# ARPA-SIMC/CRITERIA3D

Measured on AMD Instinct MI355X. Metric: simulated-hours/sec on 512x512x20 grid, higher is better.
Workload: dtype f64

## Files before the change

### criteria3d_amd/csrc/sf3d_control.inc

```

#define SYS_STORE(p, x) __hip_atomic_store((p), (x), __ATOMIC_RELAXED, __HIP_MEMORY_SCOPE_SYSTEM)
#define SYS_LOAD(p) __hip_atomic_load((p), __ATOMIC_RELAXED, __HIP_MEMORY_SCOPE_SYSTEM)

__device__ __forceinline__ unsigned long long rec_lo(double x, uint32_t tag) { return ((unsigned long long)__double_as_longlong(x) & 0xFFFFFFFFull) | ((unsigned long long)tag << 32); }
__device__ __forceinline__ unsigned long long rec_hi(double x, uint32_t tag) { return ((unsigned long long)__double_as_longlong(x) >> 32) | ((unsigned long long)tag << 32); }
__device__ __forceinline__ bool rec_ok(unsigned long long a, unsigned long long b, uint32_t tag) { return (uint32_t)(a >> 32) == tag && (uint32_t)(b >> 32) == tag; }
__device__ __forceinline__ double rec_value(unsigned long long a, unsigned long long b) { return __longlong_as_double((long long)((a & 0xFFFFFFFFull) | (b << 32))); }

__device__ __forceinline__ void dist_combine(double (&acc)[4], const double (&x)[4], int K, int op, bool first)
{
    if (first) { for (int k = 0; k < K; ++k) acc[k] = x[k]; return; }
    if (op == 1) { for (int k = 0; k < K; ++k) acc[k] = dmax(acc[k], x[k]); return; }
    if (op >= 2) {
        dd_merge(acc[0], acc[1], x[0], x[1]);
        if (op == 3) dd_merge(acc[2], acc[3], x[2], x[3]); else for (int k = 2; k < K; ++k) acc[k] += x[k];
        return;
    }
    for (int k = 0; k < K; ++k) acc[k] += x[k];
}
template <int K>
__device__ __forceinline__ bool dist_allgather(const DevView& v, Ctrl* c, double (&vals)[K], int op)
{
    static_assert(K >= 1 && K <= 4, "a mailbox holds four values");
    if (v.world <= 1) return true;
// ... 245 lines not shown
__device__ __forceinline__ void begin_attempt(Ctrl* c)
{
    c->dt = dmin(c->dtCurr, c->maxTimeStep);
    c->hold = c->cur;
    c->best = -1;
    c->bestMBR = NODATA_D;
    c->approx = 0;
    c->counters[0]++;
    c->stage = ST_APPROX;
}

__global__ void k_step_begin(Ctrl* c, double maxTimeStep)
{
    c->maxTimeStep = maxTimeStep;
    c->seqCount = 0;
    c->aBuf ^= 1u;
    begin_attempt(c);
}

__device__ __forceinline__ void reject_attempt(Ctrl* c)
{
    c->seSource = 2;
    c->cur = c->hold;
    begin_attempt(c);
}

#ifndef SF3D_PROBE_BUDGET
#define SF3D_PROBE_BUDGET 8u
#endif
__device__ __forceinline__ void courant_decision(Ctrl* c, double cmax)
{
// ... 172 lines not shown
```

### criteria3d_amd/csrc/sf3d_device.h

```cpp
#ifndef SF3D_DEVICE_H
#define SF3D_DEVICE_H

#include <stdint.h>

#define SF3D_SLOTS 10
#define SF3D_POOL 5
#define SF3D_BLOCK 256
#define SF3D_CHUNK 64
#define SF3D_MAX_BLOCKS 2048
#define CK_NONE 0
#define CK_MIXED 255

enum : uint8_t { LK_NONE = 0, LK_SOIL_VERT = 1, LK_SOIL_LAT = 2, LK_RUNOFF = 3, LK_INFILTRATION = 4 };

enum : uint32_t {
    ST_IDLE = 0,
    ST_ATTEMPT = 1,
    ST_APPROX = 2,
    ST_SWEEP = 3,
    ST_POST = 4,
    ST_RESTORE = 5,
    ST_ACCEPT = 6,
    ST_DONE = 7,
    ST_FAIL = 8
// ... 48 lines not shown
    double courant;
    double bestMBR;
    double bestNorm;
    double lastNorm;
    uint32_t stage, approx, iter, iterBudget;
    int32_t cur, hold, best;
    uint32_t linearValid;
    uint32_t seSource;
    uint32_t epoch;
    uint32_t distError;
    uint32_t distSilent;
    uint32_t pairRecTimeout;
    uint32_t kfEpoch, haloEpoch, haloPar; int32_t haloBuf;
    int32_t acceptBuf;
    uint32_t aBuf, acceptABuf;
    double acceptDt;
    BalanceDev curStep, prevStep, curPeriod, wholePeriod;
    uint32_t hStage, hIter, hIterBudget, hRows;
    int32_t tCur, tOld;
    uint32_t hSweepsLast, hPad;
    double dtWater;
    double hOuterDt, hOuterSum;
    double hMaxStep, hDt, hDone;
    double hCourant, hNorm;
    double hCacheDt;
    unsigned long long hNormBits;
    HeatBalanceDev heatCur, heatPrev;
    double heatPeriodSink;
    double query[2];
    uint32_t lineal;
// ... 109 lines not shown
    const uint32_t* nodeLat;
    const uint64_t* chunkCode;
    unsigned int* bar;
    unsigned long long* rec;
    unsigned long long* prec;
    unsigned long long* gpub;
    unsigned long long* prec2;
    uint32_t fusedPost;
    double* pub;
    const uint32_t* haloSrc;
    uint32_t forceTimeout;
    int32_t sidePeer[2];
    uint32_t recFast, putBase[2];
};

struct DevView {
    uint32_t N, ns, nb;
    uint32_t Nnorm;
    uint32_t nChunks;
    uint32_t qSplit;
    uint32_t nbSurf, nbSoil;
    double probeMin;
    const uint32_t* chunkList; uint32_t nList, nListSurf;
    const uint32_t* asmList;
    uint32_t pLo, pHi;
    uint32_t aLo, aHi;
    const uint32_t* bndList; uint32_t nBnd;
    const uint16_t* lmask;
    uint32_t haloDirect;
    uint32_t ntStream;
    const DistView* dist;
    int32_t world, rank;
    const uint8_t* owner;
    const ChunkDesc* cdesc;
    const double *z, *size, *pond, *sink;
    const uint16_t* cls;
    const uint8_t* btype;
    const double *bslope, *bsize, *prescribed;
    const uint32_t* lto;
    const uint8_t* lkind;
    const uint8_t* probeMask;
    const double *larea, *ldist;
    double* lflowSum;
    sf3d_d2* A2x[2];
    double *b, *C;
    double* X[SF3D_POOL];
    double *Se, *SeHold, *K, *flow, *bflowRate, *bflowSum;
    double* compatCv; uint8_t* compatCn; double* compatDiag;
    double *cgDiag, *cgR, *cgP, *cgQ;
    double *part0, *part1;
    double *part2, *part3;
    unsigned int* arrive;
    unsigned int* gridBar;
    const SoilDev* soils;
    const double* roughness;
    PairGrid pair;
    ResGrid res;
    Ctrl* ctrl;
    HeatDev heat;
// ... 262 lines not shown
```

### criteria3d_amd/csrc/sf3d_host_build.inc

```

namespace {

template <class F> void parallel_for(uint32_t n, F f)
{
    unsigned nt = std::thread::hardware_concurrency();
    if (nt == 0) nt = 1;
    if (nt > 16) nt = 16;
    if (n < 65536 || nt == 1) { f(0u, n); return; }
    std::vector<std::thread> th;
    const uint32_t chunk = (n + nt - 1) / nt;
    for (unsigned t = 0; t < nt; ++t) {
        const uint32_t a = t * chunk, b = (a + chunk < n) ? a + chunk : n;
        if (a >= b) break;
        th.emplace_back([=] { f(a, b); });
    }
    for (auto& t : th) t.join();
}

const char* kKernelNames[KID_COUNT] = {"k_props", "k_assemble", "k_sweep", "k_post", "k_restore", "k_accept", "k_sweep_pair", "k_sweep_resident", "k_output_map"};

}

sf3d_error_t sf3d_partition_bounds(uint32_t ns, int world, uint32_t* bounds)
{
// ... 130 lines not shown
    char* tables = nullptr;
    double* nodes = nullptr;
    size_t off[8] = {0};
    uint32_t nCells = 0, nrLayers = 0, nUnits = 0, nSoils = 0, nodesN = 0;
    uint64_t nodesColVer = 0;
    int32_t lastEvapLayer = 0;
    double area = 0.;
    float flag = -9999.f;
    bool computed = false;
    double lastMs = 0.;
};

struct DeviceSolver::Impl {
    int device = -1;
    hipStream_t stream = nullptr;
    hipStream_t stream2 = nullptr;
    hipEvent_t evLinks[2] = {nullptr, nullptr};
    bool linksPending[2] = {false, false};
    int overlapAccept = -1;
    DevView v{};
    Ctrl* hostCtrl = nullptr;
    std::vector<void*> allocs;
    uint32_t N = 0, ns = 0;
    uint32_t ownedNodes = 0;
    uint32_t lastSweeps = 8;
    uint32_t lastBatches = 1;
    uint32_t predCount = 0, pred[16] = {0};
    uint32_t lastHeatSweeps = 8;
    std::vector<uint32_t> gsLevelStart;
    uint32_t lastHeatSteps = 1;
    double* heatOut[6] = {nullptr};
    double* heatAirP = nullptr;
    std::vector<std::pair<uint32_t, hipGraphExec_t>> graphs;
    int useFused = -1;
// ... 45 lines not shown
        SF3D_SYM(pGroupStart, "ncclGroupStart"); SF3D_SYM(pGroupEnd, "ncclGroupEnd"); SF3D_SYM(pAllGather, "ncclAllGather");
        #undef SF3D_SYM
        return true;
    }
    void rccl_halo(hipStream_t st, int fields)
    {
        pGroupStart();
        for (int p = 0; p < hostDist.world; ++p) {
            if (p == hostDist.rank) continue;
            if (hostDist.sendCount[p]) pSend(hostDist.sendBuf[p], (size_t)hostDist.sendCount[p] * fields, ncclDouble, p, comm, st);
            if (hostDist.recvCount[p]) pRecv(const_cast<double*>(hostDist.recvBuf[p]), (size_t)hostDist.recvCount[p] * fields, ncclDouble, p, comm, st);
        }
        pGroupEnd();
    }
    void rccl_gather(hipStream_t st) { pAllGather(rcclMine, rcclGathered, 4, ncclDouble, comm, st); }
    std::vector<uint8_t> dslot;
    std::vector<double> stage;
    uint32_t connectGen = 0;
    bool warnedShared = false;
    int timing = 0;
    std::vector<std::pair<const void*, uint32_t>> residentBlocks;
    std::vector<uint32_t> propsNeed;
    hipStream_t stream3 = nullptr;
    hipEvent_t evSlab[8] = {};
    int slabs = -1; uint32_t slabPropsBlocks = 0, slabAsmBlocks = 0; double slabFirst = 0.;
    int residentGrids = -1;
    uint32_t pairBlocks = 0;
    bool pairMasked = false;
    uint32_t resBlocks = 0, resLds = 0;
    uint32_t resCapacity = 0;
// ... 37 lines not shown
    if (!impl_) impl_ = new Impl();
    int count = 0;
    HIP_TRY(hipGetDeviceCount(&count));
    if (dev < 0 || dev >= count) { snprintf(err_, sizeof(err_), "device %d out of range (%d visible)", dev, count); return SF3D_SOLVER_ERROR; }
    impl_->device = dev;
    HIP_TRY(hipSetDevice(dev));
    return SF3D_OK;
}

static uint64_t g_deviceBytes = 0;
sf3d_error_t DeviceSolver::release()
{
    if (!impl_) return SF3D_OK;
    Impl& I = *impl_;
    if (I.stream) hipStreamSynchronize(I.stream);
    if (I.stream2) hipStreamSynchronize(I.stream2);
    if (I.stream3) hipStreamSynchronize(I.stream3);
#if SF3D_RES_PROFILE
    if (built_ && I.v.res.on && I.v.res.pub) {
        double pr[32];
        if (hipMemcpy(pr, I.v.res.pub, sizeof(pr), hipMemcpyDeviceToHost) == hipSuccess && pr[16] > 0.) {
            const char* names[7] = {"compute + record stores issued", "wave sum + block partial", "halo records", "partial records of all blocks", "barrier B", "norm + decision", "(prologue: per launch, not per iteration)"};
            fprintf(stderr, "[sf3d] resident sweep loop, block 0: %.0f launches, %.2f iterations per launch, %.2f us per launch\n", pr[16], pr[15] / pr[16], pr[17] / pr[16] / 100.);
            for (int p = 0; p < 7; ++p) fprintf(stderr, "[sf3d]   %-40s %7.2f us per iteration\n", names[p], pr[8 + p] / pr[15] / 100.);
        }
    }
#endif
    I.linksPending[0] = I.linksPending[1] = false;
    if (I.stream3) {
        (void)hipStreamDestroy(I.stream3); I.stream3 = nullptr;
        for (auto& ev : I.evSlab) if (ev) { (void)hipEventDestroy(ev); ev = nullptr; }
    }
    I.slabs = -1;
    for (auto& p : I.pending) { I.freeEvents.push_back(p.a); I.freeEvents.push_back(p.b); }
    I.pending.clear();
    for (auto& g : I.graphs) hipGraphExecDestroy(g.second);
    I.graphs.clear();
    for (void* p : I.allocs) hipFree(p);
    I.allocs.clear();
    g_deviceBytes = 0;
    I.maps.free_all();
    if (I.sink.nodes) { (void)hipFree(I.sink.nodes); I.sink.nodes = nullptr; I.sink.nodesN = 0; I.sink.computed = false; }
    if (I.comm && I.pCommDestroy) { I.pCommDestroy(I.comm); I.comm = nullptr; }
// ... 1 lines not shown
    for (void* p : I.peerMaps) hipIpcCloseMemHandle(p);
    I.peerMaps.clear();
    I.drop_shm();
    if (I.window) { hipFree(I.window); I.window = nullptr; }
    I.devDist = nullptr; I.distStats = nullptr;
    connected_ = false;
    built_ = false;
    fatal_ = false;
    I.overlapAccept = I.useFused = I.useGraphs = I.residentGrids = -1;
    return SF3D_OK;
}

sf3d_error_t DeviceSolver::synchronize()
{
    if (!impl_ || !impl_->stream) return SF3D_OK;
    HIP_TRY(hipStreamSynchronize(impl_->stream));
    if (impl_->stream2) { HIP_TRY(hipStreamSynchronize(impl_->stream2)); impl_->linksPending[0] = impl_->linksPending[1] = false; }
    return SF3D_OK;
}

template <class T> static hipError_t dev_alloc(std::vector<void*>& allocs, T*& p, size_t count)
{
    void* q = nullptr;
    hipError_t e = hipMalloc(&q, (count ? count : 1) * sizeof(T));
    if (e == hipSuccess) { allocs.push_back(q); p = static_cast<T*>(q); g_deviceBytes += (uint64_t)(count ? count : 1) * sizeof(T); }
    return e;
}
uint64_t DeviceSolver::device_bytes() const { return g_deviceBytes; }

static void fill_params(Ctrl& c, const ParamsHost& p)
{
    c.MBRThreshold = p.MBRThreshold; c.residualTolerance = p.residualTolerance;
// ... 22 lines not shown
                if (pick < 0 || pick >= count) { snprintf(err_, sizeof(err_), "SF3D_DEVICES names device %d, %d visible", pick, count); return SF3D_SOLVER_ERROR; }
                dev = pick;
            }
        }
        I.device = dev % count;
    }
    HIP_TRY(hipSetDevice(I.device));
    if (!I.stream) HIP_TRY(hipStreamCreateWithFlags(&I.stream, hipStreamNonBlocking));
    return SF3D_OK;
}

sf3d_error_t DeviceSolver::sync_to_device(HostModel& m, const ParamsHost& p)
{
    { const sf3d_error_t e = ensure_device(); if (e != SF3D_OK) return e; }
    Impl& I = *impl_;
    if ((I.linksPending[0] || I.linksPending[1]) && (m.graphDirty || m.stateDirty || m.flowSumsDirty || !built_)) { HIP_TRY(hipStreamSynchronize(I.stream2)); I.linksPending[0] = I.linksPending[1] = false; }
    if (!I.hostCtrl) HIP_TRY(hipHostMalloc((void**)&I.hostCtrl, sizeof(Ctrl), hipHostMallocDefault));

    const uint32_t N = m.N, ns = m.ns;
    const size_t NS = (size_t)N * SF3D_SLOTS;

    if (m.graphDirty || !built_) {
        if (world_ > 1 && connected_) { snprintf(err_, sizeof(err_), "topology changed after sf3d_dist_connect: call sf3d_dist_prepare / export / connect again"); return SF3D_TOPOGRAPHY_ERROR; }
        if (m.surf.size() < N || m.hasClass.size() < N) { snprintf(err_, sizeof(err_), "the model's build arrays were released (a trimmed strip): re-initialise before changing the topology"); return SF3D_TOPOGRAPHY_ERROR; }
        for (uint32_t i = 0; i < N; ++i) {
            if ((m.surf[i] != 0) != (i < ns)) { snprintf(err_, sizeof(err_), "node %u: surface nodes must be exactly the first nrSurfaceNodes indices", i); return SF3D_TOPOGRAPHY_ERROR; }
            if (!m.hasClass[i]) { snprintf(err_, sizeof(err_), "node %u has no soil/surface class", i); return SF3D_MISSING_DATA_ERROR; }
        }
        if (built_) { if (m.hostStaleState) fetch_state(m); if (m.hostStaleFlows) fetch_flows(m); if (m.heat && m.hostStaleHeat && I.v.heat.on) fetch_heat(m); }
        release();
        I.N = N; I.ns = ns;
// ... 377 lines not shown
            const uint32_t per = SF3D_BLOCK / SF3D_CHUNK;
            auto blocks = [&](uint32_t chunks) { uint32_t b = (chunks + per - 1) / per; if (b > SF3D_MAX_BLOCKS) b = SF3D_MAX_BLOCKS; return b; };
            v.nbSoil = blocks(v.nList - v.nListSurf);
            if (const char* be = getenv("SF3D_ASM_SOIL_BLOCKS")) { const uint32_t nb = (uint32_t)atoi(be); if (nb > 0 && nb < v.nbSoil) v.nbSoil = nb; }
        }
        double *z, *size, *pond, *sink, *bslope, *bsize, *prescribed, *roughness, *larea, *ldist;
        uint16_t* cls; uint8_t *btype, *lkind; uint32_t* lto; SoilDev* soils; ChunkDesc* dcdesc;
        HIP_TRY(dev_alloc(I.allocs, z, N)); HIP_TRY(dev_alloc(I.allocs, size, N));
        HIP_TRY(dev_alloc(I.allocs, pond, N)); HIP_TRY(dev_alloc(I.allocs, sink, N));
        HIP_TRY(dev_alloc(I.allocs, cls, N)); HIP_TRY(dev_alloc(I.allocs, btype, N));
        HIP_TRY(dev_alloc(I.allocs, bslope, N)); HIP_TRY(dev_alloc(I.allocs, bsize, N));
        HIP_TRY(dev_alloc(I.allocs, prescribed, N));
        HIP_TRY(dev_alloc(I.allocs, lto, NS)); HIP_TRY(dev_alloc(I.allocs, lkind, NS));
        HIP_TRY(dev_alloc(I.allocs, larea, NS)); HIP_TRY(dev_alloc(I.allocs, ldist, NS));
        HIP_TRY(dev_alloc(I.allocs, v.lflowSum, NS)); HIP_TRY(dev_alloc(I.allocs, v.A2x[0], NS / 2)); HIP_TRY(dev_alloc(I.allocs, v.A2x[1], NS / 2));
        HIP_TRY(dev_alloc(I.allocs, v.b, N)); HIP_TRY(dev_alloc(I.allocs, v.C, N));
        for (int k = 0; k < SF3D_POOL; ++k) HIP_TRY(dev_alloc(I.allocs, v.X[k], N));
        HIP_TRY(dev_alloc(I.allocs, v.Se, N)); HIP_TRY(dev_alloc(I.allocs, v.K, N)); HIP_TRY(dev_alloc(I.allocs, v.SeHold, N));
        HIP_TRY(dev_alloc(I.allocs, dcdesc, (size_t)nChunks));
        uint32_t* dlist; HIP_TRY(dev_alloc(I.allocs, dlist, listSurf.size()));
        if (!listSurf.empty()) HIP_TRY(hipMemcpy(dlist, listSurf.data(), listSurf.size() * 4, hipMemcpyHostToDevice));
        v.chunkList = dlist;
        v.asmList = dlist;
        v.owner = nullptr; v.dist = nullptr;
        {
            const char* e = getenv("SF3D_NT_STREAM");
            const double sweepBytes = 152.0 * (double)v.nList * SF3D_CHUNK;
            v.ntStream = e ? (e[0] != '0') : (sweepBytes > 256.0 * 1024 * 1024);
        }
        {
// ... 566 lines not shown
                for (uint32_t i = 0; i < ns; ++i) if (kind[(size_t)sl * N + i] == LK_RUNOFF) { v.probeMin = -1.; break; }
            uint8_t* dpm; HIP_TRY(dev_alloc(I.allocs, dpm, (size_t)(ns ? ns : 1)));
            if (ns) HIP_TRY(hipMemcpy(dpm, pm.data(), ns, hipMemcpyHostToDevice));
            v.probeMask = dpm;
        }
        {   std::vector<uint16_t> mask(N, 0);
            for (int sl = 0; sl < SF3D_SLOTS; ++sl) { const uint8_t* kk = kind.data() + (size_t)sl * N; for (uint32_t i = 0; i < N; ++i) if (kk[i] != LK_NONE) mask[i] |= (uint16_t)(1u << sl); }
            uint16_t* dm; HIP_TRY(dev_alloc(I.allocs, dm, N));
            HIP_TRY(hipMemcpy(dm, mask.data(), (size_t)N * 2, hipMemcpyHostToDevice));
            v.lmask = dm; }
        HIP_TRY(hipMemcpy(larea, area.data(), NS * 8, hipMemcpyHostToDevice));
        HIP_TRY(hipMemcpy(ldist, dist.data(), NS * 8, hipMemcpyHostToDevice));
        HIP_TRY(hipMemcpy(dcdesc, cdesc.data(), cdesc.size() * sizeof(ChunkDesc), hipMemcpyHostToDevice));
        if (!sd.empty()) HIP_TRY(hipMemcpy(soils, sd.data(), sd.size() * sizeof(SoilDev), hipMemcpyHostToDevice));
        if (!m.roughness.empty()) HIP_TRY(hipMemcpy(roughness, m.roughness.data(), m.roughness.size() * 8, hipMemcpyHostToDevice));
        HIP_TRY(hipMemset(v.A2x[0], 0, NS * 8)); HIP_TRY(hipMemset(v.A2x[1], 0, NS * 8)); HIP_TRY(hipMemset(v.b, 0, N * 8)); HIP_TRY(hipMemset(v.C, 0, N * 8));
        HIP_TRY(hipMemset(v.flow, 0, N * 8)); HIP_TRY(hipMemset(v.bflowRate, 0, N * 8)); HIP_TRY(hipMemset(v.SeHold, 0, N * 8));
        for (int k = 0; k < SF3D_POOL; ++k) HIP_TRY(hipMemset(v.X[k], 0, N * 8));
        if (m.heat && I.heatAirP) hipLaunchKernelGGL(k_heat_static, dim3(v.nb), dim3(SF3D_BLOCK), 0, 0, v, I.heatAirP);
        HIP_TRY(hipDeviceSynchronize());

        std::memset(&mirror_, 0, sizeof(mirror_));
        mirror_.cur = 0; mirror_.hold = 0; mirror_.best = -1; mirror_.stage = ST_IDLE;
        mirror_.bestMBR = NODATA_D;
        mirror_.tCur = 0; mirror_.tOld = 0; mirror_.hStage = HS_IDLE;
        built_ = true;
        m.graphDirty = false;
        m.stateDirty = m.sinkDirty = m.pondDirty = m.boundaryDirty = m.flowSumsDirty = m.ctrlDirty = true;
        m.sinkLo = 0; m.sinkHi = UINT32_MAX;
        m.hostStaleState = m.hostStaleFlows = false;
    }

    DevView& v = I.v;
    if (m.stateDirty) {
        HIP_TRY(hipMemcpyAsync(v.X[mirror_.cur], m.H.data(), N * 8, hipMemcpyHostToDevice, I.stream));
        HIP_TRY(hipMemcpyAsync(v.Se, m.Se.data(), N * 8, hipMemcpyHostToDevice, I.stream));
        HIP_TRY(hipMemcpyAsync(v.K, m.K.data(), N * 8, hipMemcpyHostToDevice, I.stream));
        mirror_.seSource = 0; m.ctrlDirty = true;
        m.stateDirty = false;
    }
// ... 55 lines not shown
```

### criteria3d_amd/csrc/sf3d_host_step.inc

```
sf3d_error_t DeviceSolver::fetch_state(HostModel& m)
{
    Impl& I = *impl_;
    HIP_TRY(hipMemcpyAsync(m.H.data(), I.v.X[mirror_.cur], (size_t)m.N * 8, hipMemcpyDeviceToHost, I.stream));
    HIP_TRY(hipMemcpyAsync(m.Se.data(), I.v.Se, (size_t)m.N * 8, hipMemcpyDeviceToHost, I.stream));
    HIP_TRY(hipMemcpyAsync(m.K.data(), I.v.K, (size_t)m.N * 8, hipMemcpyDeviceToHost, I.stream));
    HIP_TRY(hipStreamSynchronize(I.stream));
    m.hostStaleState = false;
    return SF3D_OK;
}

sf3d_error_t DeviceSolver::fetch_flows(HostModel& m)
{
    Impl& I = *impl_;
    const size_t N = m.N;
    if (I.stream2) { HIP_TRY(hipStreamSynchronize(I.stream2)); I.linksPending[0] = I.linksPending[1] = false; }
    HIP_TRY(hipMemcpyAsync(m.bflowSum.data(), I.v.bflowSum, N * 8, hipMemcpyDeviceToHost, I.stream));
    HIP_TRY(hipMemcpyAsync(m.bflowRate.data(), I.v.bflowRate, N * 8, hipMemcpyDeviceToHost, I.stream));
    if (I.dslot.empty()) {
        for (int s = 0; s < SF3D_SLOTS; ++s)
            HIP_TRY(hipMemcpyAsync(m.lflowSum[s].data(), I.v.lflowSum + (size_t)s * N, N * 8, hipMemcpyDeviceToHost, I.stream));
        HIP_TRY(hipStreamSynchronize(I.stream));
    } else {
        I.stage.resize(N * SF3D_SLOTS);
        HIP_TRY(hipMemcpyAsync(I.stage.data(), I.v.lflowSum, N * SF3D_SLOTS * 8, hipMemcpyDeviceToHost, I.stream));
        HIP_TRY(hipStreamSynchronize(I.stream));
        for (int s = 0; s < SF3D_SLOTS; ++s) {
            const uint8_t* d = I.dslot.data() + (size_t)s * N; double* dst = m.lflowSum[s].data();
            for (size_t i = 0; i < N; ++i) dst[i] = I.stage[(size_t)d[i] * N + i];
        }
    }
// ... 632 lines not shown
sf3d_error_t DeviceSolver::step(HostModel& m, ParamsHost& p, double maxTimeStep, double* dtOut)
{
    RoctxRange stepRange("sf3d computeStep");
    sf3d_error_t e = sync_to_device(m, p);
    if (e != SF3D_OK) return e;
    if (world_ > 1 && !connected_) { snprintf(err_, sizeof(err_), "multi-GPU model used before sf3d_dist_connect / sf3d_dist_finalize%s%.150s", distWhy_[0] ? ": " : "", distWhy_); return SF3D_SOLVER_ERROR; }
    Impl& I = *impl_;
    const DevView& v = I.v;
    const dim3 grid(v.nb), block(SF3D_BLOCK), one(1);
    const bool multi = world_ > 1;
    const bool heatOn = v.heat.on != 0;
    if (I.useFused < 0) { const char* e = getenv("SF3D_FUSED_DECIDE"); I.useFused = (e && e[0] == '0') ? 0 : 1; }
    if (I.residentGrids < 0) { const char* e = getenv("SF3D_RESIDENT_GRIDS"); I.residentGrids = (e && e[0] == '0') ? 0 : 1; }
    const bool compat = v.compatCv != nullptr;
    auto resident = [&](const void* fn) -> dim3 {
        uint32_t nbk = 0;
        for (auto& r : I.residentBlocks) if (r.first == fn) nbk = r.second;
        if (nbk == 0) {
            int perCu = 0, dev = 0; hipDeviceProp_t prop;
            nbk = SF3D_MAX_BLOCKS;
            if (hipOccupancyMaxActiveBlocksPerMultiprocessor(&perCu, fn, SF3D_BLOCK, 0) == hipSuccess && perCu > 0
                && hipGetDevice(&dev) == hipSuccess && hipGetDeviceProperties(&prop, dev) == hipSuccess && prop.multiProcessorCount > 0)
                nbk = (uint32_t)perCu * (uint32_t)prop.multiProcessorCount;
            if (I.residentGrids == 0) nbk = SF3D_MAX_BLOCKS;
            I.residentBlocks.push_back({fn, nbk});
        }
        return dim3(v.nb < nbk ? v.nb : nbk);
    };
    if (heatOn && multi) I.useFused = 1;
    const bool fused = !multi && I.useFused;
    const bool fusedMulti = multi && I.useFused;
    const bool linealOn = p.lineal && v.cgDiag != nullptr && !multi && I.useFused;
    const bool resOn = v.res.on && I.resBlocks != 0 && (fused || (fusedMulti && v.haloDirect && !I.rcclMode)) && !linealOn;
    if (resOn && !multi) {
        static const long failAt = getenv("SF3D_RESIDENT_FAIL_TEST") ? strtol(getenv("SF3D_RESIDENT_FAIL_TEST"), nullptr, 10) : -1;
        I.v.res.forceTimeout = (failAt >= 0 && (long)I.stepSeqAll == failAt) ? 1u : 0u;
        ++I.stepSeqAll;
    }
    const bool pairOn = !resOn && (fused || (fusedMulti && v.haloDirect && v.nBnd != 0)) && I.pairBlocks != 0 && !linealOn;
    const dim3 pgrid(I.pushBlocks ? I.pushBlocks : 1);
    hipStream_t st = I.stream;

    const bool timedStep = I.timing == 1 || (I.timing == 2 && (I.stepSeq++ % 8 == 0));
    if (I.overlapAccept < 0) { const char* oe = getenv("SF3D_OVERLAP_ACCEPT"); I.overlapAccept = (oe && oe[0] == '0') ? 0 : 1; }
    if (I.overlapAccept && !multi && !I.stream2) { HIP_TRY(hipStreamCreateWithFlags(&I.stream2, hipStreamNonBlocking)); HIP_TRY(hipEventCreateWithFlags(&I.evLinks[0], hipEventDisableTiming)); HIP_TRY(hipEventCreateWithFlags(&I.evLinks[1], hipEventDisableTiming)); }
    const bool overlap = I.overlapAccept && !multi && I.stream2 && !timedStep && I.timing != 1 && v.compatCv == nullptr;
    auto timed = [&](int kid, auto launch) {
        if (!timedStep || (I.timing == 2 && kid != KID_SWEEP && kid != KID_SWEEP_PAIR && kid != KID_SWEEP_RES)) { launch(); return; }
        hipEvent_t a, b;
        if (I.freeEvents.size() >= 2) { a = I.freeEvents.back(); I.freeEvents.pop_back(); b = I.freeEvents.back(); I.freeEvents.pop_back(); }
        else { hipEventCreate(&a); hipEventCreate(&b); }
        hipEventRecord(a, st); launch(); hipEventRecord(b, st);
        I.pending.push_back({a, b, kid});
    };

    if (heatOn) {
        if (v.heat.save == 2) hipLaunchKernelGGL(k_heat_reset_water_fluxes, grid, block, 0, st, v);
        hipLaunchKernelGGL(k_heat_conductance, grid, block, 0, st, v);
        for (int t = 0; t < SF3D_FLUX_TYPES; ++t) m.lfluxValid[t] = false;
    }
    uint32_t stage = ST_ACCEPT;
    if (m.water) {
    {
        const uint32_t wb = (mirror_.aBuf ^ 1u) & 1u;
        if (I.linksPending[wb]) { HIP_TRY(hipStreamWaitEvent(st, I.evLinks[wb], 0)); I.linksPending[wb] = false; }
        if (!overlap && I.linksPending[wb ^ 1u]) { HIP_TRY(hipStreamWaitEvent(st, I.evLinks[wb ^ 1u], 0)); I.linksPending[wb ^ 1u] = false; }
    }
    {
    hipLaunchKernelGGL(k_step_begin, one, one, 0, st, v.ctrl, maxTimeStep);
    stage = ST_APPROX;
    uint64_t before[8], atStart[8];
    std::memcpy(before, mirror_.counters, sizeof(before));
    std::memcpy(atStart, mirror_.counters, sizeof(atStart));
    int guard = 0;
    uint64_t pairBefore = mirror_.pairLaunches, singleBefore = mirror_.singleLaunches, earlyBefore = mirror_.earlyCourant, resBefore = mirror_.residentLaunches;


    const dim3 propsGrid = resident((const void*)k_props<0, false>), propsHeatGrid = resident((const void*)k_props<0, true>);
    const dim3 acceptGrid = v.ntStream ? resident((const void*)k_accept<true>) : resident((const void*)k_accept<false>);
    auto enqueue_props = [&] {
            if (heatOn && multi) {
// ... 266 lines not shown
        pairBefore = c.pairLaunches; singleBefore = c.singleLaunches; earlyBefore = c.earlyCourant; resBefore = c.residentLaunches;

        stage = c.stage;
        if (stage != ST_SWEEP && c.iter > 0) I.lastSweeps = c.iter;
        if (stage == ST_ACCEPT || stage == ST_FAIL) break;
        if (++guard > 1000000) { snprintf(err_, sizeof(err_), "step state machine did not terminate (stage %u)", stage); return SF3D_SOLVER_ERROR; }
    }
    {
        const uint64_t used = I.hostCtrl->counters[2] - atStart[2];
        I.lastBatches = used < 1 ? 1u : (uint32_t)used;
        I.predCount = I.hostCtrl->seqCount < 16u ? I.hostCtrl->seqCount : 16u;
        for (uint32_t k = 0; k < I.predCount; ++k) I.pred[k] = I.hostCtrl->seqSweeps[k];
    }
    }
    if (overlap && stage == ST_ACCEPT) {
        uint32_t lcap = 384u; if (const char* le = getenv("SF3D_LINKS_BLOCKS")) lcap = (uint32_t)atoi(le);
        const dim3 lgrid(v.nb > lcap ? lcap : v.nb);
        const Ctrl& hc = *I.hostCtrl;
        const uint32_t rb = hc.acceptABuf & 1u;
        if (v.ntStream) hipLaunchKernelGGL(k_accept_links<true>, lgrid, block, 0, I.stream2, v, hc.acceptBuf, rb, hc.acceptDt);
        else hipLaunchKernelGGL(k_accept_links<false>, lgrid, block, 0, I.stream2, v, hc.acceptBuf, rb, hc.acceptDt);
        HIP_TRY(hipEventRecord(I.evLinks[rb], I.stream2));
        I.linksPending[rb] = true;
    }
    }

    if (heatOn && stage == ST_ACCEPT) {
        hipLaunchKernelGGL(k_heat_begin, one, one, 0, st, v.ctrl, maxTimeStep, m.water ? 1 : 0);
        const dim3 gSaveWater = v.ntStream ? resident((const void*)k_heat_save_water<true>) : resident((const void*)k_heat_save_water<false>), gBoundary = resident((const void*)k_heat_boundary),
                   gHProps = resident((const void*)k_heat_props), gHAsm = v.ntStream ? resident((const void*)k_heat_assemble<true>) : resident((const void*)k_heat_assemble<false>),
                   gHPost = resident((const void*)k_heat_post), gHSave = resident((const void*)k_heat_save);
        hipLaunchKernelGGL(k_heat_save_water_props, resident((const void*)k_heat_save_water_props), block, 0, st, v);
        if (v.ntStream) hipLaunchKernelGGL(k_heat_save_water<true>, gSaveWater, block, 0, st, v); else hipLaunchKernelGGL(k_heat_save_water<false>, gSaveWater, block, 0, st, v);
        int hguard = 0;
        uint32_t lookH = I.lastHeatSteps < 1 ? 1 : (I.lastHeatSteps > 8 ? 8 : I.lastHeatSteps);
        if (v.heat.gs) lookH = 1;
        if (I.useGraphs < 0) { const char* e = getenv("SF3D_GRAPHS"); I.useGraphs = (e && e[0] == '0') ? 0 : 1; }
        auto enqueue_heat = [&](uint32_t steps, uint32_t chunk) {
// ... 92 lines not shown
```

### criteria3d_amd/csrc/sf3d_maps.inc

```

#define MAP_GRAVITY 9.80665
#define MAP_NODATA (-9999.0)
enum : int32_t {
    MV_VWC = 0, MV_TOTAL_POTENTIAL = 1, MV_MATRIC_POTENTIAL = 2, MV_AVAILABLE_WATER = 3, MV_DEGREE_OF_SATURATION = 4, MV_AVG_DEGREE_OF_SATURATION = 5,
    MV_WATER_DEFICIT = 9, MV_WATER_INFLOW = 10, MV_WATER_OUTFLOW = 11, MV_FACTOR_OF_SAFETY = 12, MV_MINIMUM_FACTOR_OF_SAFETY = 13,
    MV_SURFACE_POND = 14, MV_MIN_VWC = 15, MV_MAX_VWC = 16
};

__device__ __forceinline__ double map_theta(const SoilDev& s, double Se) { return (Se * (s.thetaS - s.thetaR)) + s.thetaR; }
__device__ __forceinline__ double map_theta_at(const SoilDev& s, double absPsi, uint32_t wrc) { return map_theta(s, se_from_psi(s, absPsi, wrc)); }

__device__ __forceinline__ double map_node_value(const MapView& m, int32_t var, uint32_t i)
{
    const bool surf = i < m.ns;
    switch (var) {
        case MV_VWC: return surf ? (m.H[i] - m.z[i]) : map_theta(m.soils[m.cls[i]], m.Se[i]);
        case MV_TOTAL_POTENTIAL: return m.H[i];
        case MV_MATRIC_POTENTIAL: return m.H[i] - m.z[i];
        case MV_AVAILABLE_WATER: {
            if (surf) return m.H[i] - m.z[i];
            const SoilDev& s = m.soils[m.cls[i]];
            return dmax(0., map_theta(s, m.Se[i]) - map_theta_at(s, 160., m.wrc));
        }
        case MV_DEGREE_OF_SATURATION: {
// ... 149 lines not shown
        HIP_TRY(maps_reserve(C.slope, C.slopeCap, 2 * cells));
        HIP_TRY(hipMemcpyAsync(C.slope, in.slope, 2 * cells * 8, hipMemcpyHostToDevice, I.stream));
        C.slopeVer = in.slopeVer;
    }
    if (C.geoHost.size() != in.nGeo || (in.nGeo && std::memcmp(C.geoHost.data(), in.geo, in.nGeo * sizeof(MapGeo)) != 0)) {
        C.geoHost.assign(in.geo, in.geo + in.nGeo);
        HIP_TRY(maps_reserve(C.geo, C.geoCap, in.nGeo));
        HIP_TRY(hipMemcpyAsync(C.geo, C.geoHost.data(), in.nGeo * sizeof(MapGeo), hipMemcpyHostToDevice, I.stream));
    }
    const bool whole = var == MV_MINIMUM_FACTOR_OF_SAFETY || var == MV_AVG_DEGREE_OF_SATURATION;
    const uint32_t lay0 = whole ? 0u : (layer < 0 ? 0u : (uint32_t)layer), lay1 = whole ? 1u : (layer < 0 ? in.nLayers : (uint32_t)layer + 1);
    const size_t outN = (size_t)(lay1 - lay0) * cells;
    HIP_TRY(maps_reserve(C.out, C.outCap, outN));
    if (!C.missing) HIP_TRY(hipMalloc((void**)&C.missing, sizeof(int)));
    HIP_TRY(hipMemsetAsync(C.missing, 0, sizeof(int), I.stream));
    if ((var == MV_WATER_INFLOW || var == MV_WATER_OUTFLOW) && I.stream2) HIP_TRY(hipStreamSynchronize(I.stream2));

    MapView mv{};
    mv.col = C.col; mv.thick = C.thick; mv.slope = C.slope; mv.geo = C.geo;
    mv.H = I.v.X[mirror_.cur]; mv.Se = I.v.Se; mv.z = I.v.z; mv.pond = I.v.pond; mv.lflowSum = I.v.lflowSum;
    mv.cls = I.v.cls; mv.soils = I.v.soils;
    mv.N = I.v.N; mv.ns = I.v.ns; mv.nCells = in.nCells; mv.nLayers = in.nLayers; mv.lay0 = lay0; mv.lay1 = lay1; mv.wrc = p.wrc;
    mv.var = var; mv.flag = flag; mv.out = C.out; mv.missing = C.missing;
    const dim3 grid((in.nCells + SF3D_BLOCK - 1) / SF3D_BLOCK);
    hipEvent_t ev[2] = {nullptr, nullptr};
    if (I.timing) { HIP_TRY(hipEventCreate(&ev[0])); HIP_TRY(hipEventCreate(&ev[1])); HIP_TRY(hipEventRecord(ev[0], I.stream)); }
    if (in.nCells) hipLaunchKernelGGL(k_output_map, grid, dim3(SF3D_BLOCK), 0, I.stream, mv);
    HIP_TRY(hipGetLastError());
    if (I.timing) HIP_TRY(hipEventRecord(ev[1], I.stream));
    HIP_TRY(hipMemcpyAsync(out, C.out, outN * sizeof(float), hipMemcpyDeviceToHost, I.stream));
    int miss = 0;
// ... 84 lines not shown
```

### criteria3d_amd/csrc/sf3d_phases.inc

```

#define FOR_EACH_CHUNK_OF(list, l0, l1)                                                           \
    const uint32_t lane_ = threadIdx.x & 63u;                                                     \
    const uint32_t wavesTotal_ = gridDim.x * (SF3D_BLOCK / 64);                                   \
    for (uint32_t li_ = __builtin_amdgcn_readfirstlane((l0) + blockIdx.x * (SF3D_BLOCK / 64) + (threadIdx.x >> 6)); \
         li_ < (l1); li_ += wavesTotal_)                                                          \
        for (uint32_t q = __builtin_amdgcn_readfirstlane((list)[li_]), once_ = 1; once_; once_ = 0)
#define FOR_EACH_CHUNK_IN(v, l0, l1) FOR_EACH_CHUNK_OF((v).chunkList, l0, l1)
#define FOR_EACH_CHUNK(v) FOR_EACH_CHUNK_IN(v, 0u, (v).nList)
#define NOT_MINE(v, i) ((i) >= (v).N || ((v).owner != nullptr && (v).owner[i] != (v).rank))

#include "sf3d_heat.inc"

template <bool HEAT>
__device__ __forceinline__ double boundary_update(const DevView& v, const Ctrl* c, uint32_t i, double H, double Ho,
                                                  double z, double K, double Se)
{
    const double dt = c->dt;
    double flow = v.sink[i];
    if (i < v.ns && flow < 0) {
        const double avgH = 0.5 * (H + Ho);
        const double hs = dmax(0., avgH - z);
        const double maxFlux = -hs * v.size[i] / dt;
        flow = dmax(flow, maxFlux);
    }
// ... 839 lines not shown
    }
}
template <bool NT>
__global__ void __launch_bounds__(SF3D_BLOCK) k_accept(DevView v)
{
    if (v.ctrl->stage != ST_ACCEPT) return;
    body_accept<NT>(v);
}


__global__ void __launch_bounds__(SF3D_BLOCK) k_accept_boundary(DevView v)
{
    const Ctrl* c = v.ctrl;
    if (c->stage != ST_ACCEPT) return;
    const double dt = c->dt;
    FOR_EACH_CHUNK(v) {
        const uint32_t i = q * SF3D_CHUNK + lane_;
        if (NOT_MINE(v, i)) continue;
        if (v.btype[i] != SF3D_BND_NONE) v.bflowSum[i] += v.bflowRate[i] * dt;
    }
}
template <bool NT>
__global__ void __launch_bounds__(SF3D_BLOCK) k_accept_links(DevView v, int xbuf, uint32_t abuf, double dt)
{
    const double* __restrict__ X = v.X[xbuf];
    const sf3d_d2* __restrict__ A2 = v.A2x[abuf & 1u];
    FOR_EACH_CHUNK(v) {
        const uint32_t i = q * SF3D_CHUNK + lane_;
        if (NOT_MINE(v, i)) continue;
        accept_links_row<NT>(v, A2, q, i, X, dt);
    }
}

__global__ void __launch_bounds__(SF3D_BLOCK) k_storage(DevView v)
{
    const Ctrl* c = v.ctrl;
    const double* __restrict__ Xc = v.X[c->cur];
    double st = 0.;
    FOR_EACH_CHUNK(v) {
        const uint32_t i = q * SF3D_CHUNK + lane_;
        if (NOT_MINE(v, i)) continue;
        const double H = Xc[i], z = v.z[i];
        double theta;
        if (i >= v.ns) { const SoilDev s = v.soils[v.cls[i]]; theta = (v.Se[i] * (s.thetaS - s.thetaR)) + s.thetaR; }
        else theta = dmax(H - z, 0.0);
// ... 7 lines not shown
```

### criteria3d_amd/csrc/sf3d_physics.inc

```

typedef double sf3d_v2 __attribute__((ext_vector_type(2)));
template <bool NT> __device__ __forceinline__ sf3d_d2 load_coeff(const sf3d_d2* p)
{
    sf3d_v2 t;
    if (NT) t = __builtin_nontemporal_load(reinterpret_cast<const sf3d_v2*>(p));
    else t = *reinterpret_cast<const sf3d_v2*>(p);
    sf3d_d2 r; r.x = t.x; r.y = t.y; return r;
}
template <bool NT> __device__ __forceinline__ void store_coeff(sf3d_d2* p, double x, double y)
{
    sf3d_v2 t; t.x = x; t.y = y;
    if (NT) __builtin_nontemporal_store(t, reinterpret_cast<sf3d_v2*>(p));
    else *reinterpret_cast<sf3d_v2*>(p) = t;
}
typedef float sf3d_fv2 __attribute__((ext_vector_type(2)));
template <bool NT> __device__ __forceinline__ sf3d_f2 load_f2(const sf3d_f2* p)
{
    sf3d_fv2 t;
    if (NT) t = __builtin_nontemporal_load(reinterpret_cast<const sf3d_fv2*>(p));
    else t = *reinterpret_cast<const sf3d_fv2*>(p);
    sf3d_f2 r; r.x = t.x; r.y = t.y; return r;
}
template <bool NT> __device__ __forceinline__ void store_f2(sf3d_f2* p, float x, float y)
{
// ... 90 lines not shown
#else
    return __ocml_powr_f64(x, y);
#endif
}
__device__ __forceinline__ double pcbrt(double x)
{
#if SF3D_FAST_POW
    return sf3d_fcbrt(x);
#else
    return cbrt(x);
#endif
}
__device__ __forceinline__ double tortuosity(double Se, double L) { return (L == 0.5) ? sqrt(Se) : ppow(Se, L); }
#endif

__device__ __forceinline__ sf3d_d2* cur_A2(const DevView& v) { return v.A2x[v.ctrl->aBuf & 1u]; }

__device__ __forceinline__ int free_buffer3(int cur, int hold, int best)
{
    for (int b = 0; b < SF3D_POOL; ++b)
        if (b != cur && b != hold && b != best) return b;
    return 0;
}
__device__ __forceinline__ int free_buffer(const Ctrl* c) { return free_buffer3(c->cur, c->hold, c->best); }

__device__ __forceinline__ void free_buffers2(const Ctrl* c, int& f1, int& f2)
{
    uint32_t used = (1u << c->cur) | (1u << c->hold);
    if (c->best >= 0) used |= 1u << c->best;
    uint32_t fr = ~used & ((1u << SF3D_POOL) - 1u);
    f1 = __builtin_ctz(fr); fr &= fr - 1u;
// ... 145 lines not shown
```

Measured before the change: 43.75.

## Batch per-step link flow accumulation over a ring of saved matrices

Replaces the per-step link-flow accumulation kernel on a second stream with a ring of matrix and head snapshots. Accepted steps are queued on the host, and one flush kernel later walks all queued steps. Each link's running flow sum is loaded and stored once per batch instead of once per step, and the second stream with its event syncs goes away. In exchange it allocates up to eight extra matrix and head buffers, adds a copy of the head array in the boundary-accept kernel, and all flush points must be kept consistent.

```diff
diff --git a/criteria3d_amd/csrc/sf3d_control.inc b/criteria3d_amd/csrc/sf3d_control.inc
--- a/criteria3d_amd/csrc/sf3d_control.inc
+++ b/criteria3d_amd/csrc/sf3d_control.inc
@@ -283,7 +283,11 @@
 {
     c->maxTimeStep = maxTimeStep;
     c->seqCount = 0;
-    c->aBuf ^= 1u;
+    {
+        const uint32_t ring = c->aRing < 2u ? 2u : (c->aRing > (uint32_t)SF3D_LINKS_RING ? (uint32_t)SF3D_LINKS_RING : c->aRing);
+        const uint32_t nx = c->aBuf + 1u;
+        c->aBuf = nx < ring ? nx : 0u;
+    }
     begin_attempt(c);
 }
 
diff --git a/criteria3d_amd/csrc/sf3d_device.h b/criteria3d_amd/csrc/sf3d_device.h
--- a/criteria3d_amd/csrc/sf3d_device.h
+++ b/criteria3d_amd/csrc/sf3d_device.h
@@ -4,6 +4,10 @@
 #include <stdint.h>
 
 #define SF3D_SLOTS 10
+#ifndef SF3D_LINKS_RING
+#define SF3D_LINKS_RING 8
+#endif
+static_assert(SF3D_LINKS_RING >= 2 && SF3D_LINKS_RING <= 16, "the ring holds the matrix of the step in progress and at least one accepted step's");
 #define SF3D_POOL 5
 #define SF3D_BLOCK 256
 #define SF3D_CHUNK 64
@@ -86,6 +90,7 @@
     uint32_t kfEpoch, haloEpoch, haloPar; int32_t haloBuf;
     int32_t acceptBuf;
     uint32_t aBuf, acceptABuf;
+    uint32_t aRing;
     double acceptDt;
     BalanceDev curStep, prevStep, curPeriod, wholePeriod;
     uint32_t hStage, hIter, hIterBudget, hRows;
@@ -225,6 +230,8 @@
     uint32_t recFast, putBase[2];
 };
 
+struct LinksBatch { uint32_t n, slot[SF3D_LINKS_RING]; double dt[SF3D_LINKS_RING]; };
+
 struct DevView {
     uint32_t N, ns, nb;
     uint32_t Nnorm;
@@ -253,7 +260,8 @@
     const uint8_t* probeMask;
     const double *larea, *ldist;
     double* lflowSum;
-    sf3d_d2* A2x[2];
+    sf3d_d2* A2x[SF3D_LINKS_RING];
+    double* Hring[SF3D_LINKS_RING];
     double *b, *C;
     double* X[SF3D_POOL];
     double *Se, *SeHold, *K, *flow, *bflowRate, *bflowSum;
diff --git a/criteria3d_amd/csrc/sf3d_host_build.inc b/criteria3d_amd/csrc/sf3d_host_build.inc
--- a/criteria3d_amd/csrc/sf3d_host_build.inc
+++ b/criteria3d_amd/csrc/sf3d_host_build.inc
@@ -168,10 +168,9 @@
 struct DeviceSolver::Impl {
     int device = -1;
     hipStream_t stream = nullptr;
-    hipStream_t stream2 = nullptr;
-    hipEvent_t evLinks[2] = {nullptr, nullptr};
-    bool linksPending[2] = {false, false};
     int overlapAccept = -1;
+    uint32_t ring = 0;
+    LinksBatch pend{};
     DevView v{};
     Ctrl* hostCtrl = nullptr;
     std::vector<void*> allocs;
@@ -247,6 +246,30 @@
         pGroupEnd();
     }
     void rccl_gather(hipStream_t st) { pAllGather(rcclMine, rcclGathered, 4, ncclDouble, comm, st); }
+    uint32_t resident_blocks(const void* fn)
+    {
+        for (auto& r : residentBlocks) if (r.first == fn) return r.second;
+        int perCu = 0, dev = 0; hipDeviceProp_t prop;
+        uint32_t nbk = SF3D_MAX_BLOCKS;
+        if (hipOccupancyMaxActiveBlocksPerMultiprocessor(&perCu, fn, SF3D_BLOCK, 0) == hipSuccess && perCu > 0
+            && hipGetDevice(&dev) == hipSuccess && hipGetDeviceProperties(&prop, dev) == hipSuccess && prop.multiProcessorCount > 0)
+            nbk = (uint32_t)perCu * (uint32_t)prop.multiProcessorCount;
+        if (residentGrids == 0) nbk = SF3D_MAX_BLOCKS;
+        residentBlocks.push_back({fn, nbk});
+        return nbk;
+    }
+    hipError_t flush_links()
+    {
+        if (pend.n == 0) return hipSuccess;
+        const void* fn = v.ntStream ? (const void*)k_links_flush<true> : (const void*)k_links_flush<false>;
+        const uint32_t nbk = resident_blocks(fn);
+        const dim3 fgrid(v.nb < nbk ? v.nb : nbk);
+        if (v.ntStream) hipLaunchKernelGGL(k_links_flush<true>, fgrid, dim3(SF3D_BLOCK), 0, stream, v, pend);
+        else hipLaunchKernelGGL(k_links_flush<false>, fgrid, dim3(SF3D_BLOCK), 0, stream, v, pend);
+        pend.n = 0;
+        return hipGetLastError();
+    }
+    bool links_pending(uint32_t slot) const { for (uint32_t k = 0; k < pend.n; ++k) if (pend.slot[k] == slot) return true; return false; }
     std::vector<uint8_t> dslot;
     std::vector<double> stage;
     uint32_t connectGen = 0;
@@ -314,7 +337,6 @@
     if (!impl_) return SF3D_OK;
     Impl& I = *impl_;
     if (I.stream) hipStreamSynchronize(I.stream);
-    if (I.stream2) hipStreamSynchronize(I.stream2);
     if (I.stream3) hipStreamSynchronize(I.stream3);
 #if SF3D_RES_PROFILE
     if (built_ && I.v.res.on && I.v.res.pub) {
@@ -326,7 +348,7 @@
         }
     }
 #endif
-    I.linksPending[0] = I.linksPending[1] = false;
+    I.pend.n = 0; I.ring = 0;
     if (I.stream3) {
         (void)hipStreamDestroy(I.stream3); I.stream3 = nullptr;
         for (auto& ev : I.evSlab) if (ev) { (void)hipEventDestroy(ev); ev = nullptr; }
@@ -358,8 +380,8 @@
 sf3d_error_t DeviceSolver::synchronize()
 {
     if (!impl_ || !impl_->stream) return SF3D_OK;
+    if (built_) HIP_TRY(impl_->flush_links());
     HIP_TRY(hipStreamSynchronize(impl_->stream));
-    if (impl_->stream2) { HIP_TRY(hipStreamSynchronize(impl_->stream2)); impl_->linksPending[0] = impl_->linksPending[1] = false; }
     return SF3D_OK;
 }
 
@@ -412,7 +434,7 @@
 {
     { const sf3d_error_t e = ensure_device(); if (e != SF3D_OK) return e; }
     Impl& I = *impl_;
-    if ((I.linksPending[0] || I.linksPending[1]) && (m.graphDirty || m.stateDirty || m.flowSumsDirty || !built_)) { HIP_TRY(hipStreamSynchronize(I.stream2)); I.linksPending[0] = I.linksPending[1] = false; }
+    if (I.pend.n && built_ && (m.graphDirty || m.stateDirty || m.flowSumsDirty)) HIP_TRY(I.flush_links());
     if (!I.hostCtrl) HIP_TRY(hipHostMalloc((void**)&I.hostCtrl, sizeof(Ctrl), hipHostMallocDefault));
 
     const uint32_t N = m.N, ns = m.ns;
@@ -820,6 +842,25 @@
         HIP_TRY(dev_alloc(I.allocs, lto, NS)); HIP_TRY(dev_alloc(I.allocs, lkind, NS));
         HIP_TRY(dev_alloc(I.allocs, larea, NS)); HIP_TRY(dev_alloc(I.allocs, ldist, NS));
         HIP_TRY(dev_alloc(I.allocs, v.lflowSum, NS)); HIP_TRY(dev_alloc(I.allocs, v.A2x[0], NS / 2)); HIP_TRY(dev_alloc(I.allocs, v.A2x[1], NS / 2));
+        {
+            const char* oe = getenv("SF3D_OVERLAP_ACCEPT");
+            I.overlapAccept = (oe && oe[0] == '0') ? 0 : 1;
+            I.ring = 0; I.pend.n = 0;
+            if (I.overlapAccept && world_ == 1 && !m.compat) {
+                const size_t keep = I.allocs.size(); const uint64_t bytesBefore = g_deviceBytes;
+                bool ok = true;
+                for (int k = 2; k < SF3D_LINKS_RING && ok; ++k) ok = dev_alloc(I.allocs, v.A2x[k], NS / 2) == hipSuccess;
+                for (int k = 0; k < SF3D_LINKS_RING && ok; ++k) ok = dev_alloc(I.allocs, v.Hring[k], N) == hipSuccess;
+                if (ok) I.ring = SF3D_LINKS_RING;
+                else {
+                    (void)hipGetLastError();
+                    while (I.allocs.size() > keep) { (void)hipFree(I.allocs.back()); I.allocs.pop_back(); }
+                    g_deviceBytes = bytesBefore;
+                    for (int k = 2; k < SF3D_LINKS_RING; ++k) v.A2x[k] = nullptr;
+                    for (int k = 0; k < SF3D_LINKS_RING; ++k) v.Hring[k] = nullptr;
+                }
+            }
+        }
         HIP_TRY(dev_alloc(I.allocs, v.b, N)); HIP_TRY(dev_alloc(I.allocs, v.C, N));
         for (int k = 0; k < SF3D_POOL; ++k) HIP_TRY(dev_alloc(I.allocs, v.X[k], N));
         HIP_TRY(dev_alloc(I.allocs, v.Se, N)); HIP_TRY(dev_alloc(I.allocs, v.K, N)); HIP_TRY(dev_alloc(I.allocs, v.SeHold, N));
@@ -1416,7 +1457,9 @@
         HIP_TRY(hipMemcpy(dcdesc, cdesc.data(), cdesc.size() * sizeof(ChunkDesc), hipMemcpyHostToDevice));
         if (!sd.empty()) HIP_TRY(hipMemcpy(soils, sd.data(), sd.size() * sizeof(SoilDev), hipMemcpyHostToDevice));
         if (!m.roughness.empty()) HIP_TRY(hipMemcpy(roughness, m.roughness.data(), m.roughness.size() * 8, hipMemcpyHostToDevice));
-        HIP_TRY(hipMemset(v.A2x[0], 0, NS * 8)); HIP_TRY(hipMemset(v.A2x[1], 0, NS * 8)); HIP_TRY(hipMemset(v.b, 0, N * 8)); HIP_TRY(hipMemset(v.C, 0, N * 8));
+        for (uint32_t k = 0; k < (I.ring ? I.ring : 2u); ++k) HIP_TRY(hipMemset(v.A2x[k], 0, NS * 8));
+        for (uint32_t k = 0; k < I.ring; ++k) HIP_TRY(hipMemset(v.Hring[k], 0, N * 8));
+        HIP_TRY(hipMemset(v.b, 0, N * 8)); HIP_TRY(hipMemset(v.C, 0, N * 8));
         HIP_TRY(hipMemset(v.flow, 0, N * 8)); HIP_TRY(hipMemset(v.bflowRate, 0, N * 8)); HIP_TRY(hipMemset(v.SeHold, 0, N * 8));
         for (int k = 0; k < SF3D_POOL; ++k) HIP_TRY(hipMemset(v.X[k], 0, N * 8));
         if (m.heat && I.heatAirP) hipLaunchKernelGGL(k_heat_static, dim3(v.nb), dim3(SF3D_BLOCK), 0, 0, v, I.heatAirP);
@@ -1426,6 +1469,7 @@
         mirror_.cur = 0; mirror_.hold = 0; mirror_.best = -1; mirror_.stage = ST_IDLE;
         mirror_.bestMBR = NODATA_D;
         mirror_.tCur = 0; mirror_.tOld = 0; mirror_.hStage = HS_IDLE;
+        mirror_.aRing = I.ring ? I.ring : 2u;
         built_ = true;
         m.graphDirty = false;
         m.stateDirty = m.sinkDirty = m.pondDirty = m.boundaryDirty = m.flowSumsDirty = m.ctrlDirty = true;
diff --git a/criteria3d_amd/csrc/sf3d_host_step.inc b/criteria3d_amd/csrc/sf3d_host_step.inc
--- a/criteria3d_amd/csrc/sf3d_host_step.inc
+++ b/criteria3d_amd/csrc/sf3d_host_step.inc
@@ -13,7 +13,7 @@
 {
     Impl& I = *impl_;
     const size_t N = m.N;
-    if (I.stream2) { HIP_TRY(hipStreamSynchronize(I.stream2)); I.linksPending[0] = I.linksPending[1] = false; }
+    HIP_TRY(I.flush_links());
     HIP_TRY(hipMemcpyAsync(m.bflowSum.data(), I.v.bflowSum, N * 8, hipMemcpyDeviceToHost, I.stream));
     HIP_TRY(hipMemcpyAsync(m.bflowRate.data(), I.v.bflowRate, N * 8, hipMemcpyDeviceToHost, I.stream));
     if (I.dslot.empty()) {
@@ -676,17 +676,7 @@
     if (I.residentGrids < 0) { const char* e = getenv("SF3D_RESIDENT_GRIDS"); I.residentGrids = (e && e[0] == '0') ? 0 : 1; }
     const bool compat = v.compatCv != nullptr;
     auto resident = [&](const void* fn) -> dim3 {
-        uint32_t nbk = 0;
-        for (auto& r : I.residentBlocks) if (r.first == fn) nbk = r.second;
-        if (nbk == 0) {
-            int perCu = 0, dev = 0; hipDeviceProp_t prop;
-            nbk = SF3D_MAX_BLOCKS;
-            if (hipOccupancyMaxActiveBlocksPerMultiprocessor(&perCu, fn, SF3D_BLOCK, 0) == hipSuccess && perCu > 0
-                && hipGetDevice(&dev) == hipSuccess && hipGetDeviceProperties(&prop, dev) == hipSuccess && prop.multiProcessorCount > 0)
-                nbk = (uint32_t)perCu * (uint32_t)prop.multiProcessorCount;
-            if (I.residentGrids == 0) nbk = SF3D_MAX_BLOCKS;
-            I.residentBlocks.push_back({fn, nbk});
-        }
+        const uint32_t nbk = I.resident_blocks(fn);
         return dim3(v.nb < nbk ? v.nb : nbk);
     };
     if (heatOn && multi) I.useFused = 1;
@@ -704,9 +694,7 @@
     hipStream_t st = I.stream;
 
     const bool timedStep = I.timing == 1 || (I.timing == 2 && (I.stepSeq++ % 8 == 0));
-    if (I.overlapAccept < 0) { const char* oe = getenv("SF3D_OVERLAP_ACCEPT"); I.overlapAccept = (oe && oe[0] == '0') ? 0 : 1; }
-    if (I.overlapAccept && !multi && !I.stream2) { HIP_TRY(hipStreamCreateWithFlags(&I.stream2, hipStreamNonBlocking)); HIP_TRY(hipEventCreateWithFlags(&I.evLinks[0], hipEventDisableTiming)); HIP_TRY(hipEventCreateWithFlags(&I.evLinks[1], hipEventDisableTiming)); }
-    const bool overlap = I.overlapAccept && !multi && I.stream2 && !timedStep && I.timing != 1 && v.compatCv == nullptr;
+    const bool overlap = I.overlapAccept && !multi && I.ring && !timedStep && I.timing != 1 && v.compatCv == nullptr;
     auto timed = [&](int kid, auto launch) {
         if (!timedStep || (I.timing == 2 && kid != KID_SWEEP && kid != KID_SWEEP_PAIR && kid != KID_SWEEP_RES)) { launch(); return; }
         hipEvent_t a, b;
@@ -724,9 +712,8 @@
     uint32_t stage = ST_ACCEPT;
     if (m.water) {
     {
-        const uint32_t wb = (mirror_.aBuf ^ 1u) & 1u;
-        if (I.linksPending[wb]) { HIP_TRY(hipStreamWaitEvent(st, I.evLinks[wb], 0)); I.linksPending[wb] = false; }
-        if (!overlap && I.linksPending[wb ^ 1u]) { HIP_TRY(hipStreamWaitEvent(st, I.evLinks[wb ^ 1u], 0)); I.linksPending[wb ^ 1u] = false; }
+        const uint32_t ringSlots = mirror_.aRing < 2u ? 2u : mirror_.aRing;
+        if (I.pend.n && (!overlap || I.links_pending((mirror_.aBuf + 1u) % ringSlots))) HIP_TRY(I.flush_links());
     }
     {
     hipLaunchKernelGGL(k_step_begin, one, one, 0, st, v.ctrl, maxTimeStep);
@@ -1023,14 +1010,9 @@
     }
     }
     if (overlap && stage == ST_ACCEPT) {
-        uint32_t lcap = 384u; if (const char* le = getenv("SF3D_LINKS_BLOCKS")) lcap = (uint32_t)atoi(le);
-        const dim3 lgrid(v.nb > lcap ? lcap : v.nb);
         const Ctrl& hc = *I.hostCtrl;
-        const uint32_t rb = hc.acceptABuf & 1u;
-        if (v.ntStream) hipLaunchKernelGGL(k_accept_links<true>, lgrid, block, 0, I.stream2, v, hc.acceptBuf, rb, hc.acceptDt);
-        else hipLaunchKernelGGL(k_accept_links<false>, lgrid, block, 0, I.stream2, v, hc.acceptBuf, rb, hc.acceptDt);
-        HIP_TRY(hipEventRecord(I.evLinks[rb], I.stream2));
-        I.linksPending[rb] = true;
+        if (I.pend.n >= (uint32_t)SF3D_LINKS_RING) HIP_TRY(I.flush_links());
+        I.pend.slot[I.pend.n] = hc.acceptABuf < (uint32_t)SF3D_LINKS_RING ? hc.acceptABuf : 0u; I.pend.dt[I.pend.n] = hc.acceptDt; ++I.pend.n;
     }
     }
 
diff --git a/criteria3d_amd/csrc/sf3d_maps.inc b/criteria3d_amd/csrc/sf3d_maps.inc
--- a/criteria3d_amd/csrc/sf3d_maps.inc
+++ b/criteria3d_amd/csrc/sf3d_maps.inc
@@ -187,7 +187,7 @@
     HIP_TRY(maps_reserve(C.out, C.outCap, outN));
     if (!C.missing) HIP_TRY(hipMalloc((void**)&C.missing, sizeof(int)));
     HIP_TRY(hipMemsetAsync(C.missing, 0, sizeof(int), I.stream));
-    if ((var == MV_WATER_INFLOW || var == MV_WATER_OUTFLOW) && I.stream2) HIP_TRY(hipStreamSynchronize(I.stream2));
+    if (var == MV_WATER_INFLOW || var == MV_WATER_OUTFLOW) HIP_TRY(I.flush_links());
 
     MapView mv{};
     mv.col = C.col; mv.thick = C.thick; mv.slope = C.slope; mv.geo = C.geo;
diff --git a/criteria3d_amd/csrc/sf3d_phases.inc b/criteria3d_amd/csrc/sf3d_phases.inc
--- a/criteria3d_amd/csrc/sf3d_phases.inc
+++ b/criteria3d_amd/csrc/sf3d_phases.inc
@@ -877,21 +877,57 @@
     const Ctrl* c = v.ctrl;
     if (c->stage != ST_ACCEPT) return;
     const double dt = c->dt;
+    const double* __restrict__ X = v.X[c->cur];
+    double* __restrict__ Hk = v.Hring[c->aBuf];
     FOR_EACH_CHUNK(v) {
         const uint32_t i = q * SF3D_CHUNK + lane_;
         if (NOT_MINE(v, i)) continue;
+        Hk[i] = X[i];
         if (v.btype[i] != SF3D_BND_NONE) v.bflowSum[i] += v.bflowRate[i] * dt;
     }
 }
+template <bool NT, int S0, int H>
+__device__ __forceinline__ void links_flush_slots(const DevView& v, const LinksBatch& b, const ChunkDesc& cd, uint32_t i)
+{
+    static_assert(S0 % 2 == 0 && H % 2 == 0 && S0 + H <= SF3D_SLOTS, "whole (2p, 2p+1) pairs of A2x");
+    uint32_t j[H];
+    double f[H];
+    uint32_t touched = 0u;
+    #pragma unroll
+    for (int t = 0; t < H; ++t) {
+        const int s = S0 + t;
+        if (cd.kind[s] != CK_MIXED) j[t] = i + cd.delta[s];
+        else if ((cd.sweepUniform >> s) & 1u) { const uint32_t jj = i + (uint32_t)cd.delta[s]; j[t] = jj < v.N ? jj : i; }
+        else j[t] = v.lto[(size_t)s * v.N + i];
+        f[t] = load_stream<NT>(&v.lflowSum[(size_t)s * v.N + i]);
+    }
+    for (uint32_t k = 0; k < b.n; ++k) {
+        const sf3d_d2* __restrict__ A2 = v.A2x[b.slot[k]];
+        const double* __restrict__ X = v.Hring[b.slot[k]];
+        const double dt = b.dt[k];
+        double a[H], xj[H];
+        #pragma unroll
+        for (int p = 0; p < H / 2; ++p) { const sf3d_d2 t2 = load_coeff<NT>(&A2[(size_t)(S0 / 2 + p) * v.N + i]); a[2 * p] = t2.x; a[2 * p + 1] = t2.y; }
+        const double Hi = X[i];
+        #pragma unroll
+        for (int t = 0; t < H; ++t) xj[t] = X[j[t]];
+        #pragma unroll
+        for (int t = 0; t < H; ++t)
+            if (a[t] != 0.) { f[t] = f[t] + a[t] * (Hi - xj[t]) * dt; touched |= 1u << t; }
+    }
+    #pragma unroll
+    for (int t = 0; t < H; ++t)
+        if ((touched >> t) & 1u) store_stream<NT>(&v.lflowSum[(size_t)(S0 + t) * v.N + i], f[t]);
+}
 template <bool NT>
-__global__ void __launch_bounds__(SF3D_BLOCK) k_accept_links(DevView v, int xbuf, uint32_t abuf, double dt)
-{
-    const double* __restrict__ X = v.X[xbuf];
-    const sf3d_d2* __restrict__ A2 = v.A2x[abuf & 1u];
+__global__ void __launch_bounds__(SF3D_BLOCK) k_links_flush(DevView v, LinksBatch b)
+{
     FOR_EACH_CHUNK(v) {
         const uint32_t i = q * SF3D_CHUNK + lane_;
         if (NOT_MINE(v, i)) continue;
-        accept_links_row<NT>(v, A2, q, i, X, dt);
+        const ChunkDesc cd = v.cdesc[q];
+        links_flush_slots<NT, 0, 4>(v, b, cd, i);
+        links_flush_slots<NT, 4, SF3D_SLOTS - 4>(v, b, cd, i);
     }
 }
 
diff --git a/criteria3d_amd/csrc/sf3d_physics.inc b/criteria3d_amd/csrc/sf3d_physics.inc
--- a/criteria3d_amd/csrc/sf3d_physics.inc
+++ b/criteria3d_amd/csrc/sf3d_physics.inc
@@ -128,7 +128,7 @@
 __device__ __forceinline__ double tortuosity(double Se, double L) { return (L == 0.5) ? sqrt(Se) : ppow(Se, L); }
 #endif
 
-__device__ __forceinline__ sf3d_d2* cur_A2(const DevView& v) { return v.A2x[v.ctrl->aBuf & 1u]; }
+__device__ __forceinline__ sf3d_d2* cur_A2(const DevView& v) { return v.A2x[v.ctrl->aBuf]; }
 
 __device__ __forceinline__ int free_buffer3(int cur, int hold, int best)
 {
```

New measurement: 45.07, median of 6. 3.0% higher.
